# callmeray/PointMVSNet

Hardware: NVIDIA H100
Metric: PointFlow iters/sec (higher is better)
Workload: dtype f32

## Files before the change

include/pmvs_b200.h:

```cpp
#ifndef PMVS_B200_H_
#define PMVS_B200_H_

#include <stddef.h>
#include <stdint.h>

#ifdef __cplusplus
extern "C" {
#endif

#define PMVS_OK 0
#define PMVS_ERR_ARG 1
#define PMVS_ERR_CUDA 2
#define PMVS_ERR_WORKSPACE 3

#define PMVS_NUM_HYP 5
#define PMVS_FEAT_CH 136
#define PMVS_KNN 16
#define PMVS_MAX_VIEWS 12

typedef void* pmvs_stream_t;

int pmvs_version(void);
const char* pmvs_last_error(void);
unsigned long long pmvs_launch_count(void);

int pmvs_set_gemm_mode(int mode);
int pmvs_get_gemm_mode(void);

#define PMVS_OPT_EDGE 1
#define PMVS_OPT_KNN 2
#define PMVS_OPT_FETCH 3
#define PMVS_OPT_GEMM 4
#define PMVS_OPT_DEBUG_IDX 5
#define PMVS_OPT_GEMM_STRICT 6
int pmvs_set_option(int key, int value);
int pmvs_get_option(int key);

int pmvs_profile_enable(int on);
int pmvs_profile_collect(char* names, size_t names_bytes, float* ms, int max_records);

int pmvs_gather_knn_forward(const float* input, const int64_t* index, float* output,
                            int B, int C, int N, int K, pmvs_stream_t stream);
int pmvs_gather_knn_backward(const float* grad_output, const int64_t* index, float* grad_input,
                             int B, int C, int N, int K, pmvs_stream_t stream);
size_t pmvs_gather_knn_backward_det_workspace_bytes(int B, int N, int K);
int pmvs_gather_knn_backward_det(const float* grad_output, const int64_t* index, float* grad_input,
                                 int B, int C, int N, int K, void* workspace, size_t workspace_bytes,
                                 pmvs_stream_t stream);

// ... 20 lines not shown
                     int groups, int rows_per_group, int N, int K, int cin, int cout,
                     pmvs_stream_t stream);

size_t pmvs_edgeconv_pm_backward_workspace_bytes(int B, int N, int K, int cin, int cout);
int pmvs_edgeconv_pm_backward(const float* x, int ldx, const int32_t* idx32, const int64_t* idx64,
                              const float* w12, const float* gamma, const float* beta, float eps,
                              int concat_central, int bn_train, const float* le, const double* stats,
                              const float* dy, int lddy, float* dx, int lddx, float* dw12,
                              float* dgamma, float* dbeta, void* workspace, size_t workspace_bytes,
                              int B, int N, int K, int cin, int cout, pmvs_stream_t stream);

int pmvs_linear_pm(const float* x, int ldx, const float* w, float* y, int ldy, int groups,
                   int rows_per_group, int cin, int cout, const double* in_stats,
                   const float* in_gamma, const float* in_beta, double in_count, float eps,
                   double* out_stats, pmvs_stream_t stream);

typedef struct pmvs_flow_weights {
  const float* ec_w12[3];
  const float* ec_gamma[3];
  const float* ec_beta[3];
  const float* mlp_w[4];
  const float* mlp_gamma[3];
  const float* mlp_beta[3];
  float* ec_run_mean[3];
  float* ec_run_var[3];
  float* mlp_run_mean[3];
  float* mlp_run_var[3];
  float momentum;
  float eps;
  long long* ec_nbt[3];
// ... 34 lines not shown
```

pointmvsnet_b200/_lib.py:

```python
import ctypes as C
import os

import torch

_HERE = os.path.dirname(os.path.abspath(__file__))
LIB_PATH = os.path.join(_HERE, "libpmvs_b200.so")

if not os.path.exists(LIB_PATH):
    raise ImportError(
        "pointmvsnet_b200: %s is missing -- build it with pointmvsnet_b200/csrc/build.sh "
        "(nvcc, sm_90a).  There is no CPU fallback." % LIB_PATH)

lib = C.CDLL(LIB_PATH)

c_float_p = C.c_void_p
c_stream = C.c_void_p


class FlowWeights(C.Structure):
    _fields_ = [
        ("ec_w12", C.c_void_p * 3), ("ec_gamma", C.c_void_p * 3), ("ec_beta", C.c_void_p * 3),
        ("mlp_w", C.c_void_p * 4), ("mlp_gamma", C.c_void_p * 3), ("mlp_beta", C.c_void_p * 3),
        ("ec_run_mean", C.c_void_p * 3), ("ec_run_var", C.c_void_p * 3),
        ("mlp_run_mean", C.c_void_p * 3), ("mlp_run_var", C.c_void_p * 3),
# ... 31 lines not shown
_sig("pmvs_gather_knn_forward", I, [P, P, P, I, I, I, I, P])
_sig("pmvs_gather_knn_backward", I, [P, P, P, I, I, I, I, P])
_sig("pmvs_gather_knn_backward_det_workspace_bytes", C.c_size_t, [I, I, I])
_sig("pmvs_gather_knn_backward_det", I, [P, P, P, I, I, I, I, P, C.c_size_t, P])
_sig("pmvs_knn3d", I, [P, P, P, I, I, I, I, I, I, P])
_sig("pmvs_feature_fetch", I, [P, P, P, P, P, I, I, I, I, I, I, P])
_sig("pmvs_feature_fetch_backward", I, [P, P, P, P, P, I, I, I, I, I, I, P])
_sig("pmvs_cost_volume", I, [P, P, P, P, C.c_size_t, I, I, I, I, I, I, I, P])
_sig("pmvs_transpose", I, [P, P, I, I, I, P])
_sig("pmvs_idx64_to_idx32", I, [P, P, LL, P])
_sig("pmvs_edgeconv_pm", I, [P, I, P, P, P, P, F, I, I, P, I, P, P, I, I, I, I, I, I, P])
_sig("pmvs_edgeconv_pm_backward_workspace_bytes", C.c_size_t, [I, I, I, I, I])
_sig("pmvs_edgeconv_pm_backward", I, [P, I, P, P, P, P, P, F, I, I, P, P, P, I, P, I, P, P, P, P, C.c_size_t,
                                      I, I, I, I, I, P])
_sig("pmvs_linear_pm", I, [P, I, P, P, I, I, I, I, I, P, P, P, C.c_double, F, P, P])
_sig("pmvs_point_flow_workspace_bytes", C.c_size_t, [C.POINTER(FlowShape)])
_sig("pmvs_point_flow_iter", I, [C.POINTER(FlowShape), C.POINTER(FlowWeights), C.POINTER(C.c_void_p * 3),
                                 P, P, P, P, P, P, P, P, C.c_size_t, P])
_sig("pmvs_pyramid_to_channels_last", I, [P, P, I, I, I, I, P])
_sig("pmvs_point_flow_debug_offsets", I, [C.POINTER(FlowShape), C.POINTER(C.c_size_t * 10)])

EXPORTED = [
    "pmvs_version", "pmvs_last_error", "pmvs_launch_count", "pmvs_set_option", "pmvs_get_option", "pmvs_profile_enable", "pmvs_profile_collect", "pmvs_set_gemm_mode", "pmvs_get_gemm_mode", "pmvs_gather_knn_forward",
    "pmvs_gather_knn_backward", "pmvs_gather_knn_backward_det_workspace_bytes", "pmvs_gather_knn_backward_det", "pmvs_knn3d", "pmvs_feature_fetch", "pmvs_feature_fetch_backward",
    "pmvs_cost_volume", "pmvs_transpose", "pmvs_idx64_to_idx32", "pmvs_edgeconv_pm", "pmvs_edgeconv_pm_backward_workspace_bytes", "pmvs_edgeconv_pm_backward", "pmvs_linear_pm", "pmvs_point_flow_workspace_bytes",
    "pmvs_point_flow_iter", "pmvs_pyramid_to_channels_last", "pmvs_point_flow_debug_offsets",
]


def check(rc):
    if rc != 0:
        raise RuntimeError("libpmvs_b200: " + lib.pmvs_last_error().decode("utf-8", "replace"))


def stream_ptr():
    return torch.cuda.current_stream().cuda_stream


def ptr(t):
    return None if t is None else t.data_ptr()
# ... 19 lines not shown
    lib.pmvs_profile_enable(1 if on else 0)


def profile_collect(max_records=65536):
    names = C.create_string_buffer(max_records * 24)
    ms = (C.c_float * max_records)()
    n = lib.pmvs_profile_collect(names, len(names), C.cast(ms, C.c_void_p), max_records)
    nm = names.value.decode().split("\n")[:n]
    return [(nm[i], float(ms[i])) for i in range(n)]


def set_gemm_mode(mode):
    check(lib.pmvs_set_gemm_mode(int(mode)))


OPTIONS = {"edge": 1, "knn": 2, "fetch": 3, "gemm": 4, "debug_idx": 5, "gemm_strict": 6}


def set_option(name, value):
    check(lib.pmvs_set_option(OPTIONS[name], int(value)))


def get_option(name):
    return int(lib.pmvs_get_option(OPTIONS[name]))


def _options_from_env():
    spec = os.environ.get("PMVS_OPTIONS", "")
    for item in spec.split(","):
        if "=" in item:
            k, v = item.split("=", 1)
# ... 5 lines not shown
```

pointmvsnet_b200/csrc/api.cu:

```cuda
#include <algorithm>
#include <atomic>
#include <cstdarg>
#include <mutex>
#include <vector>

#include "common.cuh"

namespace pmvs {

static thread_local char g_err[512] = "";
static std::atomic<unsigned long long> g_launches{0};

void set_error(const char* fmt, ...) {
  va_list ap;
  va_start(ap, fmt);
  vsnprintf(g_err, sizeof(g_err), fmt, ap);
  va_end(ap);
}
void count_launch(int n) { g_launches.fetch_add((unsigned long long)n, std::memory_order_relaxed); }

static std::atomic<int> g_opt[OPT_COUNT];
static struct OptDefaults {
  OptDefaults() {
    g_opt[OPT_EDGE].store(1);
    g_opt[OPT_KNN].store(1);
    g_opt[OPT_FETCH].store(1);
    g_opt[OPT_GEMM].store(3);
  }
} g_opt_defaults;
int opt(int key) { return (key >= 0 && key < OPT_COUNT) ? g_opt[key].load(std::memory_order_relaxed) : 0; }

struct ProfRec {
  const char* name;
  cudaEvent_t a, b;
};
static std::mutex g_prof_mu;
static std::vector<ProfRec> g_prof;
static std::atomic<int> g_prof_on{0};
static thread_local int g_prof_open = -1;

void prof_begin(const char* what, cudaStream_t st) {
  if (!g_prof_on.load(std::memory_order_relaxed)) return;
// ... 73 lines not shown
    if (j >= 0 && j < N) atomicAdd(gin + t * N + j, gout[o]);
  }
}

static inline size_t align_up(size_t x) { return (x + 255) & ~(size_t)255; }

struct FlowPlan {
  int S, hs, ws, N;
  int sub_begin;
  size_t R;
  size_t cam, feature, xyz, idx, le, ecat, h0, h1, h2, stats, total;
  size_t warp_src;
  size_t cand;
  size_t st_ec[3], st_ecn[3], st_mlp[3];
  size_t st_ticket;
  size_t stats_doubles;
  size_t coef;
};

static int make_plan(const pmvs_flow_shape* s, FlowPlan& p) {
  PMVS_REQUIRE(s != nullptr, "point_flow: NULL shape");
  PMVS_REQUIRE(s->B > 0 && s->V > 0 && s->V <= PMVS_MAX_VIEWS, "point_flow: B=%d V=%d (V <= %d)", s->B, s->V,
               PMVS_MAX_VIEWS);
  PMVS_REQUIRE(s->ratio >= 1 && s->flow_h > 0 && s->flow_w > 0, "point_flow: bad flow size / ratio");
  PMVS_REQUIRE(s->flow_h % s->ratio == 0 && s->flow_w % s->ratio == 0,
               "point_flow: flow size %dx%d not divisible by ratio %d", s->flow_h, s->flow_w, s->ratio);
  PMVS_REQUIRE(s->prev_h > 0 && s->prev_w > 0, "point_flow: bad previous depth size");
  for (int l = 0; l < 3; ++l) PMVS_REQUIRE(s->pyr_h[l] > 0 && s->pyr_w[l] > 0, "point_flow: bad pyramid size");
  PMVS_REQUIRE(s->flow_h > 1 && s->flow_w > 1, "point_flow: flow size must be > 1");
  const int s_all = s->ratio * s->ratio;
// ... 17 lines not shown
  p.ecat = o; o += align_up(p.R * 224 * 4);
  p.h0 = o; o += align_up(p.R * 64 * 4);
  p.h1 = o; o += align_up(p.R * 64 * 4);
  p.h2 = o; o += align_up(p.R * 16 * 4);
  p.warp_src = o; o += align_up(warp_source_bytes(s->B, s->V, s->flow_h, s->flow_w));
  p.cand = o; o += align_up(p.R * PMVS_KNN * 2);
  size_t d = 0;
  const int ec_cout[3] = {32, 32, 64};
  const int mlp_cout[3] = {64, 64, 16};
  for (int l = 0; l < 3; ++l) {
    p.st_ec[l] = d; d += (size_t)p.S * 4 * ec_cout[l];
    p.st_ecn[l] = d; d += (size_t)p.S * 2 * ec_cout[l];
  }
  for (int l = 0; l < 3; ++l) { p.st_mlp[l] = d; d += (size_t)p.S * 2 * mlp_cout[l]; }
  p.st_ticket = d; d += (3 * (size_t)p.S + 1) / 2 + 1;
  p.stats_doubles = d;
  p.stats = o; o += align_up(d * 8);
  p.coef = o; o += align_up(3 * (size_t)p.S * 6 * 64 * sizeof(float));
  p.total = o;
  return PMVS_OK;
}

}

using namespace pmvs;

extern "C" int pmvs_version(void) { return 100; }
extern "C" const char* pmvs_last_error(void) { return g_err; }
extern "C" unsigned long long pmvs_launch_count(void) { return g_launches.load(); }

// ... 92 lines not shown
    return PMVS_ERR_CUDA;
  }
  GemmArgs g{};
  g.x = x; g.ldx = ldx; g.w = w12; g.y = le_scratch; g.ldy = 2 * cout;
  g.groups = groups; g.rows_per_group = rows_per_group; g.cin = cin; g.cout = 2 * cout; g.eps = eps;
  PMVS_TRY(launch_gemm(g, st));
  EdgeArgs e{};
  e.le = le_scratch; e.idx = idx32; e.stats = stats_scratch; e.gamma = gamma; e.beta = beta; e.eps = eps;
  e.concat_central = concat_central; e.out = out; e.ldo = ldo; e.groups = groups;
  e.rows_per_group = rows_per_group; e.N = N; e.K = K; e.cout = cout;
  if (bn_train) PMVS_TRY(launch_edge_stats(e, st));
  PMVS_TRY(launch_edge_apply(e, st));
  return PMVS_OK;
}

extern "C" int pmvs_linear_pm(const float* x, int ldx, const float* w, float* y, int ldy, int groups,
                              int rows_per_group, int cin, int cout, const double* in_stats, const float* in_gamma,
                              const float* in_beta, double in_count, float eps, double* out_stats,
                              pmvs_stream_t stream) {
  PMVS_REQUIRE(x && w && y, "linear_pm: NULL pointer");
  PMVS_REQUIRE(groups > 0 && rows_per_group > 0 && cin > 0 && cout > 0, "linear_pm: bad sizes");
  PMVS_REQUIRE(in_stats == nullptr || (in_gamma && in_beta && in_count > 0), "linear_pm: incomplete input BN");
  GemmArgs g{};
  g.x = x; g.ldx = ldx; g.w = w; g.y = y; g.ldy = ldy; g.groups = groups; g.rows_per_group = rows_per_group;
  g.cin = cin; g.cout = cout; g.in_stats = in_stats; g.in_gamma = in_gamma; g.in_beta = in_beta;
  g.in_count = in_count; g.eps = eps; g.out_stats = out_stats;
  return launch_gemm(g, (cudaStream_t)stream);
}

extern "C" size_t pmvs_point_flow_workspace_bytes(const pmvs_flow_shape* shape) {
  FlowPlan p;
  if (make_plan(shape, p) != PMVS_OK) return 0;
  return p.total;
}

extern "C" int pmvs_point_flow_debug_offsets(const pmvs_flow_shape* shape, size_t off[10]) {
  FlowPlan p;
  PMVS_TRY(make_plan(shape, p));
  off[0] = p.feature; off[1] = p.xyz; off[2] = p.idx; off[3] = p.ecat; off[4] = p.h2;
  off[5] = p.le; off[6] = p.stats; off[7] = p.total;
  off[8] = p.cand;
  off[9] = (opt(OPT_EDGE) == 0 || opt(OPT_DEBUG_IDX) != 0) ? 1 : 0;
// ... 16 lines not shown
  PMVS_REQUIRE(((uintptr_t)workspace & 255) == 0, "point_flow: workspace must be 256-byte aligned");
  cudaStream_t st = (cudaStream_t)stream;
  char* ws = (char*)workspace;
  float* cam = (float*)(ws + p.cam);
  float* feature = (float*)(ws + p.feature);
  float* xyz = (float*)(ws + p.xyz);
  int32_t* idx = (int32_t*)(ws + p.idx);
  float* le = (float*)(ws + p.le);
  float* ecat = (float*)(ws + p.ecat);
  float* h0 = (float*)(ws + p.h0);
  float* h1 = (float*)(ws + p.h1);
  float* h2 = (float*)(ws + p.h2);
  double* stats = (double*)(ws + p.stats);
  const int B = shape->B, S = p.S;
  const int rows_per_group = B * p.N;

  if (cudaMemsetAsync(stats, 0, p.stats_doubles * sizeof(double), st) != cudaSuccess) {
    set_error("point_flow: memset failed");
    return PMVS_ERR_CUDA;
  }
  const float kscale = shape->is_test ? shape->image_scale : (float)(4.0 * (double)shape->image_scale);
  PMVS_TRY(launch_cam_setup(cam_params, interval, mean, stdv, cam, B, shape->V, kscale, shape->interval_scale, st));

  float* warp_src = (float*)(ws + p.warp_src);
  PMVS_TRY(launch_warp_source(pyramids_cl, shape->pyr_h, shape->pyr_w, warp_src, B, shape->V, shape->flow_h,
                              shape->flow_w, st));
  FusedFetchParams f{};
  f.src = warp_src;
  f.depth_prev = depth_prev; f.cam_blocks = cam; f.feature = feature; f.xyz = xyz;
  f.B = B; f.V = shape->V; f.h = shape->flow_h; f.w = shape->flow_w; f.hp = shape->prev_h; f.wp = shape->prev_w;
// ... 3 lines not shown
  const int edge_impl = opt(OPT_EDGE);
  unsigned short* cand = (unsigned short*)(ws + p.cand);
  if (edge_impl != 0)
    PMVS_TRY(launch_knn3d_cand(xyz, opt(OPT_DEBUG_IDX) ? idx : nullptr, cand, S * B, PMVS_NUM_HYP, p.hs, p.ws, st));
  else
    PMVS_TRY(launch_knn3d(xyz, nullptr, idx, S * B, PMVS_NUM_HYP, p.hs, p.ws, PMVS_NUM_HYP, PMVS_KNN, st));

  const int cin[3] = {136, 32, 64}, cout[3] = {32, 32, 64}, in_off[3] = {0, 0, 32}, out_off[3] = {0, 32, 96};
  for (int l = 0; l < 3; ++l) {
    GemmArgs g{};
    g.x = l == 0 ? feature : ecat + in_off[l];
    g.ldx = l == 0 ? PMVS_FEAT_CH : 224;
    g.w = wts->ec_w12[l]; g.y = le; g.ldy = 2 * cout[l];
    g.groups = S; g.rows_per_group = rows_per_group; g.cin = cin[l]; g.cout = 2 * cout[l]; g.eps = wts->eps;
    if (edge_impl != 0) g.out_stats = stats + p.st_ec[l];
    PMVS_TRY(launch_gemm(g, st));
    if (edge_impl != 0) {
      EdgeTileArgs e{};
      e.le = le; e.cand = cand; e.cstats = stats + p.st_ec[l]; e.nstats = stats + p.st_ecn[l];
      e.coef = (float*)(ws + p.coef) + (size_t)l * S * 6 * 64;
      e.ticket = (unsigned*)(stats + p.st_ticket) + (size_t)l * S;
      e.gamma = wts->ec_gamma[l]; e.beta = wts->ec_beta[l]; e.eps = wts->eps; e.concat_central = l > 0;
      e.out = ecat + out_off[l]; e.ldo = 224; e.groups = S; e.clouds_per_group = B; e.gh = p.hs; e.gw = p.ws;
      e.cout = cout[l];
      const int tile_w = edge_impl == 2 ? 16 : 8;
      PMVS_TRY(launch_edge_tile_stats(e, tile_w, st));
      PMVS_TRY(launch_edge_tile_apply(e, tile_w, st));
    } else {
      EdgeArgs e{};
      e.le = le; e.idx = idx; e.stats = stats + p.st_ec[l]; e.gamma = wts->ec_gamma[l]; e.beta = wts->ec_beta[l];
      e.eps = wts->eps; e.concat_central = l > 0; e.out = ecat + out_off[l]; e.ldo = 224; e.groups = S;
// ... 4 lines not shown
  }

  {
    const float* xin[3] = {ecat, h0, h1};
    float* yout[3] = {h0, h1, h2};
    const int mcin[3] = {224, 64, 64}, mcout[3] = {64, 64, 16};
    for (int l = 0; l < 3; ++l) {
      GemmArgs g{};
      g.x = xin[l]; g.ldx = mcin[l]; g.w = wts->mlp_w[l]; g.y = yout[l]; g.ldy = mcout[l];
      g.groups = S; g.rows_per_group = rows_per_group; g.cin = mcin[l]; g.cout = mcout[l]; g.eps = wts->eps;
      if (l > 0) {
        g.in_stats = stats + p.st_mlp[l - 1]; g.in_gamma = wts->mlp_gamma[l - 1]; g.in_beta = wts->mlp_beta[l - 1];
        g.in_count = (double)rows_per_group;
      }
      g.out_stats = stats + p.st_mlp[l];
      PMVS_TRY(launch_gemm(g, st));
    }
  }
  HeadArgs h{};
  h.h2 = h2; h.stats = stats + p.st_mlp[2]; h.gamma = wts->mlp_gamma[2]; h.beta = wts->mlp_beta[2];
  h.w3 = wts->mlp_w[3]; h.depth_prev = depth_prev; h.interval = interval; h.depth_out = depth_out;
  h.prob_out = prob_out; h.eps = wts->eps; h.interval_scale = shape->interval_scale; h.B = B; h.S = S; h.ratio = shape->ratio; h.sub_begin = p.sub_begin; h.h = shape->flow_h;
  h.w = shape->flow_w; h.hp = shape->prev_h; h.wp = shape->prev_w;
  PMVS_TRY(launch_flow_head(h, st));

  RunUpdateBatch rb{};
  rb.groups = S; rb.momentum = wts->momentum;
  for (int l = 0; l < 3; ++l) {
    if (wts->ec_run_mean[l] && wts->ec_run_var[l]) {
      const int c = cout[l];
      const double* sl = stats + p.st_ec[l];
// ... 32 lines not shown
```

pointmvsnet_b200/csrc/common.cuh:

```cuda
#pragma once
#include <cuda_runtime.h>
#include <stdint.h>
#include <stdio.h>
#include <string.h>

#include "../../include/pmvs_b200.h"

namespace pmvs {

void set_error(const char* fmt, ...);
void count_launch(int n = 1);

void prof_begin(const char* what, cudaStream_t st);
void prof_end(cudaStream_t st);

inline int check_launch(const char* what, cudaStream_t st = nullptr) {
  cudaError_t e = cudaPeekAtLastError();
  if (e != cudaSuccess) {
    cudaGetLastError();
    set_error("%s: %s", what, cudaGetErrorString(e));
    return PMVS_ERR_CUDA;
  }
  prof_end(st);
  count_launch();
// ... 32 lines not shown
typedef float2 f32x2;
__device__ __forceinline__ f32x2 pack2(float a, float b) { return make_float2(a, b); }
__device__ __forceinline__ void unpack2(f32x2 v, float& a, float& b) { a = v.x; b = v.y; }
__device__ __forceinline__ f32x2 fma2(f32x2 a, f32x2 b, f32x2 c) { return make_float2(__fmaf_rn(a.x, b.x, c.x), __fmaf_rn(a.y, b.y, c.y)); }
__device__ __forceinline__ f32x2 add2(f32x2 a, f32x2 b) { return make_float2(__fadd_rn(a.x, b.x), __fadd_rn(a.y, b.y)); }
__device__ __forceinline__ f32x2 mul2(f32x2 a, f32x2 b) { return make_float2(__fmul_rn(a.x, b.x), __fmul_rn(a.y, b.y)); }
__device__ __forceinline__ f32x2 sub2(f32x2 a, f32x2 b) { return make_float2(__fsub_rn(a.x, b.x), __fsub_rn(a.y, b.y)); }

enum {
  OPT_EDGE = 1,
  OPT_KNN = 2,
  OPT_FETCH = 3,
  OPT_GEMM = 4,
  OPT_DEBUG_IDX = 5,
  OPT_GEMM_STRICT = 6,
  OPT_COUNT = 16
};
int opt(int key);

template <typename K>
inline int ensure_dyn_smem(K kernel, int bytes, unsigned long long& done_mask, const char* what) {
  int dev = 0;
  if (cudaGetDevice(&dev) != cudaSuccess || dev < 0 || dev > 63) dev = 0;
  if (done_mask & (1ull << dev)) return PMVS_OK;
  if (cudaFuncSetAttribute(kernel, cudaFuncAttributeMaxDynamicSharedMemorySize, bytes) != cudaSuccess) {
    cudaGetLastError();
    set_error("%s: cannot reserve %d bytes of shared memory", what, bytes);
    return PMVS_ERR_CUDA;
  }
  done_mask |= 1ull << dev;
  return PMVS_OK;
}

// ... 25 lines not shown
int launch_transpose(const float* in, float* out, int batch, int R, int C, cudaStream_t st);

struct GemmArgs {
  const float* x;
  int ldx;
  const float* w;
  float* y;
  int ldy;
  int groups, rows_per_group, cin, cout;
  const double* in_stats;
  const float* in_gamma;
  const float* in_beta;
  double in_count;
  float eps;
  double* out_stats;
};
int launch_gemm(const GemmArgs& a, cudaStream_t st);
int launch_gemm_tc(const GemmArgs& a, cudaStream_t st, const char* name);
int launch_gemm_ws(const GemmArgs& a, cudaStream_t st, const char* name);

struct EdgeArgs {
  const float* le;
  const int32_t* idx;
  double* stats;
  const float* gamma;
  const float* beta;
  float eps;
  int concat_central;
  float* out;
  int ldo;
// ... 79 lines not shown
```

pointmvsnet_b200/csrc/edge_tile.cu:

```cuda
#include <algorithm>

#include "common.cuh"
#include "tensor_map.cuh"

namespace pmvs {

namespace {

constexpr int ET_THREADS = 256;
constexpr int ET_WARPS = ET_THREADS / 32;
constexpr int ET_CP = 32;
constexpr int ET_LPP = ET_CP / 4;
constexpr int ET_PPW = 32 / ET_LPP;

__device__ __forceinline__ unsigned smem_u32(const void* p) { return (unsigned)__cvta_generic_to_shared(p); }

template <int TX, int TY>
struct TileGeom {
  static constexpr int HX = TX + 4, HY = TY + 4;
  static constexpr int ROWS = PMVS_NUM_HYP * HY * HX;
  static constexpr int NPTS = PMVS_NUM_HYP * TY * TX;
  static constexpr int BYTES = ROWS * ET_CP * 4;
  static constexpr int SMEM = BYTES;
};
// ... 77 lines not shown
      loc[s] = ok ? ldg4(a.le + (cloud_base + (size_t)(s * HW + pq)) * LD + ch0 + cl) : make_float4(0.f, 0.f, 0.f, 0.f);
    {
      unsigned done = 0;
      const unsigned parity = loads & 1u;
      while (!done) {
        asm volatile(
            "{\n\t.reg .pred p;\n\t"
            "mbarrier.try_wait.parity.shared::cta.b64 p, [%1], %2;\n\t"
            "selp.u32 %0, 1, 0, p;\n\t}"
            : "=r"(done)
            : "r"(bar_addr), "r"(parity)
            : "memory");
      }
      ++loads;
    }

    uint4 nx0, nx1;
    load_codes(0, nx0, nx1);
#pragma unroll
    for (int s = 0; s < STEPS; ++s) {
      const uint4 ca = nx0, cb = nx1;
      if (s + 1 < STEPS) load_codes(s + 1, nx0, nx1);
      if (!ok) continue;
      const int n = s * HW + pq;
      const size_t row = cloud_base + (size_t)n;
      const float4 lc = loc[s];
      const bool esc = ((ca.x | ca.y | ca.z | ca.w | cb.x | cb.y | cb.z | cb.w) & 0x80008000u) != 0u;
      const float* hbase = halo + pb0 + s * LAYER;
      f32x2 o_lo = pack2(0.f, 0.f), o_hi = o_lo, A_lo = o_lo, A_hi = o_lo, c_lo = o_lo, c_hi = o_lo;
      const f32x2 l_lo = pack2(lc.x, lc.y), l_hi = pack2(lc.z, lc.w);
// ... 187 lines not shown
```

pointmvsnet_b200/csrc/gemm_ws.cu:

```cuda
#include <algorithm>
#include <type_traits>

#include "common.cuh"
#include "tensor_map.cuh"
#include "wgmma.cuh"

namespace pmvs {

namespace ws {

using namespace wg;

constexpr int NT = 128;
constexpr int KC = 32;
constexpr int PLANE_BYTES = NT * KC * 4;
constexpr int STAGE_BYTES = 2 * PLANE_BYTES;
constexpr int CONS_WARPS = 8, CONS_THREADS = CONS_WARPS * 32;
constexpr int PROD_WARPS = 8, PROD_WARP0 = CONS_WARPS, PROD_THREADS = PROD_WARPS * 32;
constexpr int THREADS = CONS_THREADS + PROD_THREADS;
constexpr int A_LD = NT * 8 / PROD_THREADS;
static_assert(A_LD * PROD_THREADS == NT * 8, "the producers share a chunk evenly");
constexpr int MAXK = 224;
constexpr int SMEM_MAX = 227 * 1024;

// ... 325 lines not shown
  static unsigned long long smem_done = 0;
  PMVS_TRY((ensure_dyn_smem(gemm_ws_kernel<COUT, IN_BN, ASYNC, NSTAGES>, SMEM_MAX, smem_done, "gemm_ws")));
  const long long tiles = (long long)a.groups * cdiv(a.rows_per_group, NT);
  const int grid = (int)std::min<long long>(tiles, sm_count());
  prof_begin(name, st);
  gemm_ws_kernel<COUT, IN_BN, ASYNC, NSTAGES><<<grid, THREADS, smem_total, st>>>(a);
  return check_launch("gemm_ws_kernel", st);
}
namespace tma {
constexpr int NT = 64;
constexpr int STAGE_BYTES = NT * KC * 4;
constexpr int CONS_THREADS = 256;
constexpr int THREADS = CONS_THREADS + 64;
constexpr int MAX_STAGES = 32, MIN_STAGES = 8;
constexpr int BN_FLOATS = (MAXK / KC) * 4 * 16;
constexpr int TAIL_BN = 0, TAIL_RED = TAIL_BN + 2 * BN_FLOATS * 4;
__host__ __device__ constexpr int tail_bar(int cout) { return TAIL_RED + 2 * 2 * cout * 8; }
__host__ __device__ constexpr int tail_bytes(int cout) { return tail_bar(cout) + 2 * MAX_STAGES * 8; }
__host__ __device__ constexpr int stages_for(int cin, int cout) {
  return (SMEM_MAX - weight_bytes(cout, (cin + KC - 1) / KC) - tail_bytes(cout)) / STAGE_BYTES < MAX_STAGES
             ? (SMEM_MAX - weight_bytes(cout, (cin + KC - 1) / KC) - tail_bytes(cout)) / STAGE_BYTES
             : MAX_STAGES;
}
}

template <int N>
__device__ __forceinline__ void reduce_scatter_round(float* sv, int lane, int m) {
  const bool up = (lane & m) != 0;
#pragma unroll
  for (int k = 0; k < N / 2; ++k) {
    const float keep = up ? sv[k + N / 2] : sv[k], send = up ? sv[k] : sv[k + N / 2];
    sv[k] = keep + __shfl_xor_sync(0xffffffffu, send, m);
  }
// ... 3 lines not shown
__global__ void __launch_bounds__(tma::THREADS, 1) gemm_tma_kernel(const __grid_constant__ CUtensorMap tmx,
                                                                   const GemmArgs a, const int wstages) {
  constexpr int NT = tma::NT, STAGE_BYTES = tma::STAGE_BYTES, CONS_THREADS = tma::CONS_THREADS;
  constexpr int MAX_STAGES = tma::MAX_STAGES, BN_FLOATS = tma::BN_FLOATS, TAIL_BN = tma::TAIL_BN, TAIL_RED = tma::TAIL_RED;
  constexpr bool STACKED = COUT <= 64;
  constexpr int W_CHUNK = 2 * COUT * 128;
  constexpr int ACC_REGS = (STACKED ? 2 * COUT : COUT) / 2;
  constexpr int BLK = COUT < 64 ? COUT : 64;
  extern __shared__ __align__(1024) unsigned char smem[];
  const uint32_t smem_base = smem_u32(smem);

  const int K = a.cin;
  const int nch = (K + KC - 1) / KC;
  const int tid = threadIdx.x, warp = __shfl_sync(0xffffffffu, tid >> 5, 0), lane = tid & 31;
  const int tpg = (a.rows_per_group + NT - 1) / NT;
  const TileRange tr = my_tiles(a.groups * tpg);
  unsigned char* tail = smem + weight_bytes(COUT, nch) + 2 * wstages * STAGE_BYTES;
  const uint32_t bar0 = smem_u32(tail + tma::tail_bar(COUT));
  auto bar_full = [&](int w, int s) { return bar0 + 8u * (uint32_t)(w * (MAX_STAGES / 2) + s); };
  auto bar_empty = [&](int w, int s) { return bar0 + 8u * (uint32_t)(MAX_STAGES + w * (MAX_STAGES / 2) + s); };

  if (tid == 0) {
    for (int w = 0; w < 2; ++w)
      for (int s = 0; s < wstages; ++s) {
        mbar_init(bar_full(w, s), 1);
        mbar_init(bar_empty(w, s), 4);
      }
    asm volatile("fence.mbarrier_init.release.cluster;" ::: "memory");
  }
  __syncthreads();

  if (warp >= CONS_THREADS / 32) {
    const int w = warp - CONS_THREADS / 32;
    if (lane == 0) {
      const uint32_t ring = smem_base + weight_bytes(COUT, nch) + w * wstages * STAGE_BYTES;
      int stage = 0;
      uint32_t phase = 0;
      for (int i = w; i < tr.count; i += 2) {
        const int t = tr.first + i, g = t / tpg, row0 = (t - g * tpg) * NT;
        for (int c = 0; c < nch; ++c) {
          mbar_wait(bar_empty(w, stage), phase ^ 1u);
          mbar_arrive_expect_tx(bar_full(w, stage), STAGE_BYTES);
          tma_load_3d(ring + stage * STAGE_BYTES, &tmx, c * KC, row0, g, bar_full(w, stage));
          if (++stage == wstages) {
            stage = 0;
            phase ^= 1u;
          }
        }
      }
    }
    return;
  }

  const int wgi = warp >> 2, wtid = tid & 127;
  const uint32_t ring = smem_base + weight_bytes(COUT, nch) + wgi * wstages * STAGE_BYTES;
  float* sBN = (float*)(tail + TAIL_BN) + wgi * BN_FLOATS;
  double* sRed = (double*)(tail + TAIL_RED) + wgi * 2 * COUT;
  for (int i = wtid; i < 2 * COUT; i += 128) sRed[i] = 0.0;
  for (int e = tid; e < COUT * nch * 8; e += CONS_THREADS) {
    const int n = e / (nch * 8), rem = e - n * (nch * 8), c = rem >> 3, pc = rem & 7;
    const int k0 = c * KC + pc * 4;
    const float4 v = k0 < K ? ldg4(a.w + (size_t)n * K + k0) : make_float4(0.f, 0.f, 0.f, 0.f);
    float4 hi, lo;
    hi.x = tf32_hi(v.x); hi.y = tf32_hi(v.y); hi.z = tf32_hi(v.z); hi.w = tf32_hi(v.w);
    lo.x = __fsub_rn(v.x, hi.x); lo.y = __fsub_rn(v.y, hi.y); lo.z = __fsub_rn(v.z, hi.z); lo.w = __fsub_rn(v.w, hi.w);
    const uint32_t dst = smem_base + c * W_CHUNK + swz128(n, pc);
    sts128(dst, hi);
    sts128(dst + COUT * 128, lo);
  }
  fence_proxy_async();
  named_bar_sync(1, CONS_THREADS);

  const int r = (warp & 3) * 16 + (lane >> 2), q = lane & 3;
  const uint32_t fbase = r * 128 + q * 4, fx = (r & 7) << 4;
  const int frow = r, fcol = 2 * q;
  const uint32_t w_base = smem_base;
  float acc[ACC_REGS];
  uint32_t fh[16], fl[16];
  const uint32_t wg_bar = 2 + wgi;

  constexpr int HC = COUT < 64 ? COUT : 64, NH = COUT / HC;
  constexpr int NV = HC / 16;
  const int kofs = ((lane >> 2) & 1) * (8 * NV / 2) + ((lane >> 3) & 1) * (8 * NV / 4) + ((lane >> 4) & 1) * (8 * NV / 8);
  double racc[NH][NV];
#pragma unroll
  for (int h = 0; h < NH; ++h)
// ... 69 lines not shown
    fence_regs(fh);
    fence_regs(fl);
    __syncwarp();
    if (lane == 0) mbar_arrive(bar_empty(wgi, stage));
  };
  auto chunk_ks = [&](int c, int m) {
    switch (min(KC, K - c * KC) / 8) {
      case 4: chunk(std::integral_constant<int, 4>(), c, m); break;
      case 3: chunk(std::integral_constant<int, 3>(), c, m); break;
      case 2: chunk(std::integral_constant<int, 2>(), c, m); break;
      default: chunk(std::integral_constant<int, 1>(), c, m); break;
    }
  };

  int cur_g = -1;
  for (int i = wgi; i < tr.count; i += 2) {
    const int t = tr.first + i;
    const int g = t / tpg, row0 = (t - g * tpg) * NT;
    const int rows_valid = min(NT, a.rows_per_group - row0);
    const size_t grow0 = (size_t)g * a.rows_per_group + row0;
    if (g != cur_g) {
      named_bar_sync(wg_bar, 128);
      if (cur_g >= 0) flush(cur_g);
      if (IN_BN) {
        const double* s = a.in_stats + (size_t)g * 2 * K;
        for (int e = wtid; e < nch * 64; e += 128) {
          const int c = e >> 6, qq = (e >> 4) & 3, k = e & 15, jh = k & 7;
          const int col = c * KC + 8 * (jh >> 1) + qq + 4 * (jh & 1);
          float val = 0.f;
          if (col < K) {
            const BnCoef bc = bn_coef(s[col], s[K + col], a.in_count, a.eps);
            const float A = __fmul_rn(bc.invstd, a.in_gamma[col]);
            val = k < 8 ? A : fmaf(-bc.mean, A, a.in_beta[col]);
          }
          sBN[e] = val;
        }
      }
      named_bar_sync(wg_bar, 128);
      cur_g = g;
    }
    const int m0 = (i >> 1) * nch;
    for (int c = 0; c < nch; ++c) chunk_ks(c, m0 + c);
    fence_regs(acc);
    const bool ok0 = frow < rows_valid, ok1 = frow + 8 < rows_valid;
    float* y0 = a.y + (grow0 + frow) * a.ldy + fcol;
    float* y1 = y0 + (size_t)8 * a.ldy;
#pragma unroll
    for (int h = 0; h < NH; ++h) {
      float sv[HC / 2];
#pragma unroll
      for (int il = 0; il < HC / 8; ++il) {
        const int ii = h * (HC / 8) + il;
        float v[4];
#pragma unroll
        for (int e = 0; e < 4; ++e) v[e] = STACKED ? acc[4 * ii + e] + acc[COUT / 2 + 4 * ii + e] : acc[4 * ii + e];
        if (ok0) *reinterpret_cast<float2*>(y0 + 8 * ii) = make_float2(v[0], v[1]);
// ... 32 lines not shown
  EncodeTiledFn enc = encode_tiled_fn();
  if (enc == nullptr) return -1;
  CUtensorMap tm;
  const cuuint64_t gdim[3] = {(cuuint64_t)a.cin, (cuuint64_t)a.rows_per_group, (cuuint64_t)a.groups};
  const cuuint64_t gstr[2] = {row_bytes, group_bytes};
  const cuuint32_t box[3] = {KC, tma::NT, 1};
  const cuuint32_t estr[3] = {1, 1, 1};
  if (enc(&tm, CU_TENSOR_MAP_DATA_TYPE_FLOAT32, 3, const_cast<float*>(a.x), gdim, gstr, box, estr,
          CU_TENSOR_MAP_INTERLEAVE_NONE, CU_TENSOR_MAP_SWIZZLE_128B, CU_TENSOR_MAP_L2_PROMOTION_L2_256B,
          CU_TENSOR_MAP_FLOAT_OOB_FILL_NONE) != CUDA_SUCCESS)
    return -1;
  const int smem_total = weight_bytes(COUT, cdiv(a.cin, KC)) + 2 * wstages * tma::STAGE_BYTES + tma::tail_bytes(COUT);
  static unsigned long long smem_done = 0;
  PMVS_TRY((ensure_dyn_smem(gemm_tma_kernel<COUT, IN_BN>, SMEM_MAX, smem_done, "gemm_tma")));
  const long long tiles = (long long)a.groups * cdiv(a.rows_per_group, tma::NT);
  const int grid = (int)std::min<long long>(tiles, sm_count());
  prof_begin(name, st);
  gemm_tma_kernel<COUT, IN_BN><<<grid, tma::THREADS, smem_total, st>>>(tm, a, wstages);
  return check_launch("gemm_tma_kernel", st);
}

template <int COUT, bool IN_BN>
static int launch_one(const GemmArgs& a, cudaStream_t st, const char* name) {
  if (opt(OPT_GEMM) == 3) {
    const int rc = launch_tma<COUT, IN_BN>(a, st, name);
    if (rc >= 0 || opt(OPT_GEMM_STRICT)) return rc;
  }
  const bool deep = a.cin <= DEEP_K;
  if (opt(OPT_GEMM) == 1)
    return deep ? launch_pf<COUT, IN_BN, 0, 4>(a, st, name) : launch_pf<COUT, IN_BN, 0, 3>(a, st, name);
  return deep ? launch_pf<COUT, IN_BN, 4, 2>(a, st, name) : launch_pf<COUT, IN_BN, 3, 2>(a, st, name);
}

// ... 28 lines not shown
```

pointmvsnet_b200/csrc/knn3d.cu:

```cuda
#include "common.cuh"

namespace pmvs {

constexpr int KNN_TX = 32, KNN_TY = 2, KNN_TD = 5;

template <int K>
__device__ __forceinline__ void knn_insert(unsigned (&kd)[K], unsigned (&ki)[K], unsigned d, unsigned j) {
  const unsigned long long key = ((unsigned long long)d << 32) | j;
#pragma unroll
  for (int p = K - 1; p > 0; --p) {
    const unsigned long long prev = ((unsigned long long)kd[p - 1] << 32) | ki[p - 1];
    const unsigned long long cur = ((unsigned long long)kd[p] << 32) | ki[p];
    const bool lt_prev = key < prev;
    const bool lt_cur = key < cur;
    kd[p] = lt_prev ? kd[p - 1] : (lt_cur ? d : kd[p]);
    ki[p] = lt_prev ? ki[p - 1] : (lt_cur ? j : ki[p]);
  }
  const unsigned long long first = ((unsigned long long)kd[0] << 32) | ki[0];
  if (key < first) {
    kd[0] = d;
    ki[0] = j;
  }
}

// ... 200 lines not shown
    const int sx = e % KM_SX;
    int r = e / KM_SX;
    const int sy = r % KM_SY;
    const int sz = r / KM_SY;
    const int gx = x0 + sx - 2, gy = y0 + sy - 2, gz = z0 + sz - 2;
    float4 v = make_float4(0.f, 0.f, 0.f, 0.f);
    if (gx >= 0 && gx < W && gy >= 0 && gy < H && gz >= 0 && gz < D) {
      const float* p = base + gz * HW + (long long)gy * W + gx;
      v.x = __ldg(p);
      v.y = __ldg(p + DHW);
      v.z = __ldg(p + 2 * DHW);
    }
    tile[e] = v;
  }
  __syncthreads();

  const int warp = tid >> 5, lane = tid & 31;
  const int tz = warp >> 1, tx = (warp & 1) * 8 + (lane & 7), ty = lane >> 3;
  const int x = x0 + tx, y = y0 + ty, z = z0 + tz;
  const bool valid = x < W && y < H && z < D;
  const float4* self = tile + ((tz + 2) * KM_SY + ty + 2) * KM_SX + tx + 2;
  const float4 c = *self;

  double L[16];
#pragma unroll 1
  for (int b = 0; b < KM_BATCHES; ++b) {
    double k[16];
    unsigned dmin = 0xffffffffu;
    const unsigned pad = c_knn_pad[b];
#pragma unroll
// ... 142 lines not shown
```

Measured before the change: 1360.

## Add PDL overlap, dynamic tile scheduling, and batched weight staging to TMA GEMM

```diff
diff --git a/include/pmvs_b200.h b/include/pmvs_b200.h
--- a/include/pmvs_b200.h
+++ b/include/pmvs_b200.h
@@ -33,6 +33,8 @@
 #define PMVS_OPT_GEMM 4
 #define PMVS_OPT_DEBUG_IDX 5
 #define PMVS_OPT_GEMM_STRICT 6
+#define PMVS_OPT_GEMM_SCHED 7
+#define PMVS_OPT_PDL 8
 int pmvs_set_option(int key, int value);
 int pmvs_get_option(int key);
 
@@ -83,6 +85,10 @@
                    int rows_per_group, int cin, int cout, const double* in_stats,
                    const float* in_gamma, const float* in_beta, double in_count, float eps,
                    double* out_stats, pmvs_stream_t stream);
+int pmvs_linear_pm_sched(const float* x, int ldx, const float* w, float* y, int ldy, int groups,
+                         int rows_per_group, int cin, int cout, const double* in_stats,
+                         const float* in_gamma, const float* in_beta, double in_count, float eps,
+                         double* out_stats, unsigned int* tile_counter, pmvs_stream_t stream);
 
 typedef struct pmvs_flow_weights {
   const float* ec_w12[3];
diff --git a/pointmvsnet_b200/_lib.py b/pointmvsnet_b200/_lib.py
--- a/pointmvsnet_b200/_lib.py
+++ b/pointmvsnet_b200/_lib.py
@@ -69,6 +69,7 @@
 _sig("pmvs_edgeconv_pm_backward", I, [P, I, P, P, P, P, P, F, I, I, P, P, P, I, P, I, P, P, P, P, C.c_size_t,
                                       I, I, I, I, I, P])
 _sig("pmvs_linear_pm", I, [P, I, P, P, I, I, I, I, I, P, P, P, C.c_double, F, P, P])
+_sig("pmvs_linear_pm_sched", I, [P, I, P, P, I, I, I, I, I, P, P, P, C.c_double, F, P, P, P])
 _sig("pmvs_point_flow_workspace_bytes", C.c_size_t, [C.POINTER(FlowShape)])
 _sig("pmvs_point_flow_iter", I, [C.POINTER(FlowShape), C.POINTER(FlowWeights), C.POINTER(C.c_void_p * 3),
                                  P, P, P, P, P, P, P, P, C.c_size_t, P])
@@ -78,7 +79,7 @@
 EXPORTED = [
     "pmvs_version", "pmvs_last_error", "pmvs_launch_count", "pmvs_set_option", "pmvs_get_option", "pmvs_profile_enable", "pmvs_profile_collect", "pmvs_set_gemm_mode", "pmvs_get_gemm_mode", "pmvs_gather_knn_forward",
     "pmvs_gather_knn_backward", "pmvs_gather_knn_backward_det_workspace_bytes", "pmvs_gather_knn_backward_det", "pmvs_knn3d", "pmvs_feature_fetch", "pmvs_feature_fetch_backward",
-    "pmvs_cost_volume", "pmvs_transpose", "pmvs_idx64_to_idx32", "pmvs_edgeconv_pm", "pmvs_edgeconv_pm_backward_workspace_bytes", "pmvs_edgeconv_pm_backward", "pmvs_linear_pm", "pmvs_point_flow_workspace_bytes",
+    "pmvs_cost_volume", "pmvs_transpose", "pmvs_idx64_to_idx32", "pmvs_edgeconv_pm", "pmvs_edgeconv_pm_backward_workspace_bytes", "pmvs_edgeconv_pm_backward", "pmvs_linear_pm", "pmvs_linear_pm_sched", "pmvs_point_flow_workspace_bytes",
     "pmvs_point_flow_iter", "pmvs_pyramid_to_channels_last", "pmvs_point_flow_debug_offsets",
 ]
 
@@ -128,7 +129,7 @@
     check(lib.pmvs_set_gemm_mode(int(mode)))
 
 
-OPTIONS = {"edge": 1, "knn": 2, "fetch": 3, "gemm": 4, "debug_idx": 5, "gemm_strict": 6}
+OPTIONS = {"edge": 1, "knn": 2, "fetch": 3, "gemm": 4, "debug_idx": 5, "gemm_strict": 6, "gemm_sched": 7, "pdl": 8}
 
 
 def set_option(name, value):
diff --git a/pointmvsnet_b200/csrc/api.cu b/pointmvsnet_b200/csrc/api.cu
--- a/pointmvsnet_b200/csrc/api.cu
+++ b/pointmvsnet_b200/csrc/api.cu
@@ -26,6 +26,8 @@
     g_opt[OPT_KNN].store(1);
     g_opt[OPT_FETCH].store(1);
     g_opt[OPT_GEMM].store(3);
+    g_opt[OPT_GEMM_SCHED].store(0);
+    g_opt[OPT_PDL].store(1);
   }
 } g_opt_defaults;
 int opt(int key) { return (key >= 0 && key < OPT_COUNT) ? g_opt[key].load(std::memory_order_relaxed) : 0; }
@@ -129,6 +131,7 @@
   size_t cand;
   size_t st_ec[3], st_ecn[3], st_mlp[3];
   size_t st_ticket;
+  size_t st_tiles;
   size_t stats_doubles;
   size_t coef;
 };
@@ -176,6 +179,7 @@
   }
   for (int l = 0; l < 3; ++l) { p.st_mlp[l] = d; d += (size_t)p.S * 2 * mlp_cout[l]; }
   p.st_ticket = d; d += (3 * (size_t)p.S + 1) / 2 + 1;
+  p.st_tiles = d; d += 3;
   p.stats_doubles = d;
   p.stats = o; o += align_up(d * 8);
   p.coef = o; o += align_up(3 * (size_t)p.S * 6 * 64 * sizeof(float));
@@ -298,18 +302,26 @@
   return PMVS_OK;
 }
 
-extern "C" int pmvs_linear_pm(const float* x, int ldx, const float* w, float* y, int ldy, int groups,
-                              int rows_per_group, int cin, int cout, const double* in_stats, const float* in_gamma,
-                              const float* in_beta, double in_count, float eps, double* out_stats,
-                              pmvs_stream_t stream) {
+extern "C" int pmvs_linear_pm_sched(const float* x, int ldx, const float* w, float* y, int ldy, int groups,
+                                    int rows_per_group, int cin, int cout, const double* in_stats,
+                                    const float* in_gamma, const float* in_beta, double in_count, float eps,
+                                    double* out_stats, unsigned int* tile_counter, pmvs_stream_t stream) {
   PMVS_REQUIRE(x && w && y, "linear_pm: NULL pointer");
   PMVS_REQUIRE(groups > 0 && rows_per_group > 0 && cin > 0 && cout > 0, "linear_pm: bad sizes");
   PMVS_REQUIRE(in_stats == nullptr || (in_gamma && in_beta && in_count > 0), "linear_pm: incomplete input BN");
   GemmArgs g{};
   g.x = x; g.ldx = ldx; g.w = w; g.y = y; g.ldy = ldy; g.groups = groups; g.rows_per_group = rows_per_group;
   g.cin = cin; g.cout = cout; g.in_stats = in_stats; g.in_gamma = in_gamma; g.in_beta = in_beta;
-  g.in_count = in_count; g.eps = eps; g.out_stats = out_stats;
+  g.in_count = in_count; g.eps = eps; g.out_stats = out_stats; g.tile_counter = tile_counter;
   return launch_gemm(g, (cudaStream_t)stream);
+}
+
+extern "C" int pmvs_linear_pm(const float* x, int ldx, const float* w, float* y, int ldy, int groups,
+                              int rows_per_group, int cin, int cout, const double* in_stats, const float* in_gamma,
+                              const float* in_beta, double in_count, float eps, double* out_stats,
+                              pmvs_stream_t stream) {
+  return pmvs_linear_pm_sched(x, ldx, w, y, ldy, groups, rows_per_group, cin, cout, in_stats, in_gamma, in_beta,
+                              in_count, eps, out_stats, nullptr, stream);
 }
 
 extern "C" size_t pmvs_point_flow_workspace_bytes(const pmvs_flow_shape* shape) {
@@ -356,6 +368,12 @@
   double* stats = (double*)(ws + p.stats);
   const int B = shape->B, S = p.S;
   const int rows_per_group = B * p.N;
+  unsigned* tile_counters = opt(OPT_GEMM_SCHED) ? (unsigned*)(stats + p.st_tiles) : nullptr;
+  auto contraction = [&](GemmArgs& g, int k) {
+    g.tile_counter = tile_counters ? tile_counters + k : nullptr;
+    g.pdl = opt(OPT_PDL);
+    return launch_gemm(g, st);
+  };
 
   if (cudaMemsetAsync(stats, 0, p.stats_doubles * sizeof(double), st) != cudaSuccess) {
     set_error("point_flow: memset failed");
@@ -389,7 +407,7 @@
     g.w = wts->ec_w12[l]; g.y = le; g.ldy = 2 * cout[l];
     g.groups = S; g.rows_per_group = rows_per_group; g.cin = cin[l]; g.cout = 2 * cout[l]; g.eps = wts->eps;
     if (edge_impl != 0) g.out_stats = stats + p.st_ec[l];
-    PMVS_TRY(launch_gemm(g, st));
+    PMVS_TRY(contraction(g, l));
     if (edge_impl != 0) {
       EdgeTileArgs e{};
       e.le = le; e.cand = cand; e.cstats = stats + p.st_ec[l]; e.nstats = stats + p.st_ecn[l];
@@ -424,7 +442,7 @@
         g.in_count = (double)rows_per_group;
       }
       g.out_stats = stats + p.st_mlp[l];
-      PMVS_TRY(launch_gemm(g, st));
+      PMVS_TRY(contraction(g, 3 + l));
     }
   }
   HeadArgs h{};
diff --git a/pointmvsnet_b200/csrc/common.cuh b/pointmvsnet_b200/csrc/common.cuh
--- a/pointmvsnet_b200/csrc/common.cuh
+++ b/pointmvsnet_b200/csrc/common.cuh
@@ -70,9 +70,14 @@
   OPT_GEMM = 4,
   OPT_DEBUG_IDX = 5,
   OPT_GEMM_STRICT = 6,
+  OPT_GEMM_SCHED = 7,
+  OPT_PDL = 8,
   OPT_COUNT = 16
 };
 int opt(int key);
+
+__device__ __forceinline__ void griddep_wait() { asm volatile("griddepcontrol.wait;" ::: "memory"); }
+__device__ __forceinline__ void griddep_launch_dependents() { asm volatile("griddepcontrol.launch_dependents;" ::: "memory"); }
 
 template <typename K>
 inline int ensure_dyn_smem(K kernel, int bytes, unsigned long long& done_mask, const char* what) {
@@ -128,6 +133,8 @@
   double in_count;
   float eps;
   double* out_stats;
+  unsigned* tile_counter;
+  int pdl;
 };
 int launch_gemm(const GemmArgs& a, cudaStream_t st);
 int launch_gemm_tc(const GemmArgs& a, cudaStream_t st, const char* name);
diff --git a/pointmvsnet_b200/csrc/edge_tile.cu b/pointmvsnet_b200/csrc/edge_tile.cu
--- a/pointmvsnet_b200/csrc/edge_tile.cu
+++ b/pointmvsnet_b200/csrc/edge_tile.cu
@@ -115,6 +115,7 @@
       }
       ++loads;
     }
+    if (APPLY && slab == SLABS - 1) griddep_launch_dependents();
 
     uint4 nx0, nx1;
     load_codes(0, nx0, nx1);
diff --git a/pointmvsnet_b200/csrc/gemm_ws.cu b/pointmvsnet_b200/csrc/gemm_ws.cu
--- a/pointmvsnet_b200/csrc/gemm_ws.cu
+++ b/pointmvsnet_b200/csrc/gemm_ws.cu
@@ -363,9 +363,12 @@
 constexpr int THREADS = CONS_THREADS + 64;
 constexpr int MAX_STAGES = 32, MIN_STAGES = 8;
 constexpr int BN_FLOATS = (MAXK / KC) * 4 * 16;
+constexpr int NO_TILE = -1;
+constexpr int MIN_TILES_PER_CTA = 16;
 constexpr int TAIL_BN = 0, TAIL_RED = TAIL_BN + 2 * BN_FLOATS * 4;
 __host__ __device__ constexpr int tail_bar(int cout) { return TAIL_RED + 2 * 2 * cout * 8; }
-__host__ __device__ constexpr int tail_bytes(int cout) { return tail_bar(cout) + 2 * MAX_STAGES * 8; }
+__host__ __device__ constexpr int tail_tile(int cout) { return tail_bar(cout) + 2 * MAX_STAGES * 8; }
+__host__ __device__ constexpr int tail_bytes(int cout) { return tail_tile(cout) + MAX_STAGES * 4; }
 __host__ __device__ constexpr int stages_for(int cin, int cout) {
   return (SMEM_MAX - weight_bytes(cout, (cin + KC - 1) / KC) - tail_bytes(cout)) / STAGE_BYTES < MAX_STAGES
              ? (SMEM_MAX - weight_bytes(cout, (cin + KC - 1) / KC) - tail_bytes(cout)) / STAGE_BYTES
@@ -399,11 +402,13 @@
   const int nch = (K + KC - 1) / KC;
   const int tid = threadIdx.x, warp = __shfl_sync(0xffffffffu, tid >> 5, 0), lane = tid & 31;
   const int tpg = (a.rows_per_group + NT - 1) / NT;
-  const TileRange tr = my_tiles(a.groups * tpg);
+  const int total_tiles = a.groups * tpg;
   unsigned char* tail = smem + weight_bytes(COUT, nch) + 2 * wstages * STAGE_BYTES;
   const uint32_t bar0 = smem_u32(tail + tma::tail_bar(COUT));
   auto bar_full = [&](int w, int s) { return bar0 + 8u * (uint32_t)(w * (MAX_STAGES / 2) + s); };
   auto bar_empty = [&](int w, int s) { return bar0 + 8u * (uint32_t)(MAX_STAGES + w * (MAX_STAGES / 2) + s); };
+  volatile int* tile_slot = reinterpret_cast<volatile int*>(tail + tma::tail_tile(COUT));
+  auto slot = [&](int w, int s) -> volatile int& { return tile_slot[w * (MAX_STAGES / 2) + s]; };
 
   if (tid == 0) {
     for (int w = 0; w < 2; ++w)
@@ -418,13 +423,25 @@
   if (warp >= CONS_THREADS / 32) {
     const int w = warp - CONS_THREADS / 32;
     if (lane == 0) {
+      asm volatile("prefetch.tensormap [%0];" ::"l"(&tmx) : "memory");
+      griddep_wait();
       const uint32_t ring = smem_base + weight_bytes(COUT, nch) + w * wstages * STAGE_BYTES;
       int stage = 0;
       uint32_t phase = 0;
-      for (int i = w; i < tr.count; i += 2) {
-        const int t = tr.first + i, g = t / tpg, row0 = (t - g * tpg) * NT;
+      const TileRange tr = my_tiles(total_tiles);
+      int i = w;
+      auto next_tile = [&]() -> int {
+        if (a.tile_counter != nullptr) return (int)atomicAdd(a.tile_counter, 1u);
+        const int t = i < tr.count ? tr.first + i : total_tiles;
+        i += 2;
+        return t;
+      };
+      for (int t = next_tile(); t < total_tiles;) {
+        const int t_next = next_tile();
+        const int g = t / tpg, row0 = (t - g * tpg) * NT;
         for (int c = 0; c < nch; ++c) {
           mbar_wait(bar_empty(w, stage), phase ^ 1u);
+          if (c == 0) slot(w, stage) = t;
           mbar_arrive_expect_tx(bar_full(w, stage), STAGE_BYTES);
           tma_load_3d(ring + stage * STAGE_BYTES, &tmx, c * KC, row0, g, bar_full(w, stage));
           if (++stage == wstages) {
@@ -432,7 +449,12 @@
             phase ^= 1u;
           }
         }
-      }
+        t = t_next;
+      }
+      mbar_wait(bar_empty(w, stage), phase ^ 1u);
+      slot(w, stage) = tma::NO_TILE;
+      mbar_arrive(bar_full(w, stage));
+      griddep_launch_dependents();
     }
     return;
   }
@@ -442,19 +464,43 @@
   float* sBN = (float*)(tail + TAIL_BN) + wgi * BN_FLOATS;
   double* sRed = (double*)(tail + TAIL_RED) + wgi * 2 * COUT;
   for (int i = wtid; i < 2 * COUT; i += 128) sRed[i] = 0.0;
-  for (int e = tid; e < COUT * nch * 8; e += CONS_THREADS) {
-    const int n = e / (nch * 8), rem = e - n * (nch * 8), c = rem >> 3, pc = rem & 7;
-    const int k0 = c * KC + pc * 4;
-    const float4 v = k0 < K ? ldg4(a.w + (size_t)n * K + k0) : make_float4(0.f, 0.f, 0.f, 0.f);
-    float4 hi, lo;
-    hi.x = tf32_hi(v.x); hi.y = tf32_hi(v.y); hi.z = tf32_hi(v.z); hi.w = tf32_hi(v.w);
-    lo.x = __fsub_rn(v.x, hi.x); lo.y = __fsub_rn(v.y, hi.y); lo.z = __fsub_rn(v.z, hi.z); lo.w = __fsub_rn(v.w, hi.w);
-    const uint32_t dst = smem_base + c * W_CHUNK + swz128(n, pc);
-    sts128(dst, hi);
-    sts128(dst + COUT * 128, lo);
+  constexpr int WB = 8;
+  const int pieces = COUT * nch * 8;
+  auto piece = [&](int e, int& n, int& c, int& pc) {
+    n = e / (nch * 8);
+    const int rem = e - n * (nch * 8);
+    c = rem >> 3;
+    pc = rem & 7;
+  };
+  for (int e0 = tid; e0 < pieces; e0 += WB * CONS_THREADS) {
+    float4 v[WB];
+#pragma unroll
+    for (int u = 0; u < WB; ++u) {
+      const int e = e0 + u * CONS_THREADS;
+      int n, c, pc;
+      piece(e, n, c, pc);
+      const int k0 = c * KC + pc * 4;
+      v[u] = e < pieces && k0 < K ? ldg4(a.w + (size_t)n * K + k0) : make_float4(0.f, 0.f, 0.f, 0.f);
+    }
+#pragma unroll
+    for (int u = 0; u < WB; ++u) {
+      const int e = e0 + u * CONS_THREADS;
+      if (e < pieces) {
+        int n, c, pc;
+        piece(e, n, c, pc);
+        float4 hi, lo;
+        hi.x = tf32_hi(v[u].x); hi.y = tf32_hi(v[u].y); hi.z = tf32_hi(v[u].z); hi.w = tf32_hi(v[u].w);
+        lo.x = __fsub_rn(v[u].x, hi.x); lo.y = __fsub_rn(v[u].y, hi.y);
+        lo.z = __fsub_rn(v[u].z, hi.z); lo.w = __fsub_rn(v[u].w, hi.w);
+        const uint32_t dst = smem_base + c * W_CHUNK + swz128(n, pc);
+        sts128(dst, hi);
+        sts128(dst + COUT * 128, lo);
+      }
+    }
   }
   fence_proxy_async();
   named_bar_sync(1, CONS_THREADS);
+  griddep_wait();
 
   const int r = (warp & 3) * 16 + (lane >> 2), q = lane & 3;
   const uint32_t fbase = r * 128 + q * 4, fx = (r & 7) << 4;
@@ -554,8 +600,11 @@
   };
 
   int cur_g = -1;
-  for (int i = wgi; i < tr.count; i += 2) {
-    const int t = tr.first + i;
+  for (int m0 = 0;; m0 += nch) {
+    const int stage0 = m0 % wstages;
+    mbar_wait(bar_full(wgi, stage0), (uint32_t)((m0 / wstages) & 1));
+    const int t = slot(wgi, stage0);
+    if (t == tma::NO_TILE) break;
     const int g = t / tpg, row0 = (t - g * tpg) * NT;
     const int rows_valid = min(NT, a.rows_per_group - row0);
     const size_t grow0 = (size_t)g * a.rows_per_group + row0;
@@ -579,7 +628,6 @@
       named_bar_sync(wg_bar, 128);
       cur_g = g;
     }
-    const int m0 = (i >> 1) * nch;
     for (int c = 0; c < nch; ++c) chunk_ks(c, m0 + c);
     fence_regs(acc);
     const bool ok0 = frow < rows_valid, ok1 = frow + 8 < rows_valid;
@@ -642,9 +690,24 @@
   static unsigned long long smem_done = 0;
   PMVS_TRY((ensure_dyn_smem(gemm_tma_kernel<COUT, IN_BN>, SMEM_MAX, smem_done, "gemm_tma")));
   const long long tiles = (long long)a.groups * cdiv(a.rows_per_group, tma::NT);
-  const int grid = (int)std::min<long long>(tiles, sm_count());
+  const int grid = (int)std::min<long long>(cdiv(tiles, tma::MIN_TILES_PER_CTA), sm_count());
+  cudaLaunchConfig_t cfg = {};
+  cfg.gridDim = dim3(grid);
+  cfg.blockDim = dim3(tma::THREADS);
+  cfg.dynamicSmemBytes = smem_total;
+  cfg.stream = st;
+  cudaLaunchAttribute attr[1];
+  attr[0].id = cudaLaunchAttributeProgrammaticStreamSerialization;
+  attr[0].val.programmaticStreamSerializationAllowed = 1;
+  cfg.attrs = attr;
+  cfg.numAttrs = a.pdl ? 1 : 0;
   prof_begin(name, st);
-  gemm_tma_kernel<COUT, IN_BN><<<grid, tma::THREADS, smem_total, st>>>(tm, a, wstages);
+  const cudaError_t e = cudaLaunchKernelEx(&cfg, gemm_tma_kernel<COUT, IN_BN>, tm, a, wstages);
+  if (e != cudaSuccess) {
+    cudaGetLastError();
+    set_error("gemm_tma_kernel: %s", cudaGetErrorString(e));
+    return PMVS_ERR_CUDA;
+  }
   return check_launch("gemm_tma_kernel", st);
 }
 
diff --git a/pointmvsnet_b200/csrc/knn3d.cu b/pointmvsnet_b200/csrc/knn3d.cu
--- a/pointmvsnet_b200/csrc/knn3d.cu
+++ b/pointmvsnet_b200/csrc/knn3d.cu
@@ -238,6 +238,7 @@
     tile[e] = v;
   }
   __syncthreads();
+  griddep_launch_dependents();
 
   const int warp = tid >> 5, lane = tid & 31;
   const int tz = warp >> 1, tx = (warp & 1) * 8 + (lane & 7), ty = lane >> 3;
```

Measured after the change: 1383 (median of 6 runs). +1.7%, better.
